# bd4sur/Nano

Hardware: AMD Instinct MI355X
Metric: decode_tokens_per_sec (higher is better)
Workload: dtype i8

## Files before the change

### include/nano_mi355x.h

```cpp
#ifndef NANO_MI355X_H
#define NANO_MI355X_H

#include <stddef.h>
#include <stdint.h>

#ifdef __cplusplus
extern "C" {
#endif

#define NANO_ARCH_NANO  0u
#define NANO_ARCH_QWEN2 2u
#define NANO_ARCH_QWEN3 3u

#define NANO_QUANT_F32 0x00u
#define NANO_QUANT_Q80 0x80u
#define NANO_QUANT_Q4K 0x42u

#define NANO_HIP_OK        0
#define NANO_HIP_EINVAL   -1
#define NANO_HIP_ERUNTIME -2
#define NANO_HIP_ENODEV   -3
#define NANO_HIP_ENOMEM   -4

#define NANO_MAX_BATCH 64u
// ... 268 lines not shown
int nano_hip_qkv_attn_fused_plan(const NanoFusedGemvDesc *qkv, const NanoAttnDecodeDesc *attn, uint32_t cus, uint32_t out[NANO_QKV_ATTN_FUSED_PLAN_WORDS]);
int nano_hip_wo_w13_fused_plan(const NanoFusedGemvDesc *wo, const NanoFusedGemvDesc *w13, uint32_t cus, uint32_t out[NANO_WO_W13_FUSED_PLAN_WORDS]);
typedef struct NanoQkvAttnFusedDesc {
    const NanoFusedGemvDesc *qkv;
    const NanoAttnDecodeDesc *attn;
    uint32_t layer1, tick0;
    const unsigned long long *hand_init;
    float *part_out;
    float *ml_out;
    uint32_t *plan_out;
    uint32_t *err_out;
} NanoQkvAttnFusedDesc;
int nano_hip_op_qkv_attn_fused(int device, const NanoQkvAttnFusedDesc *d);
typedef struct NanoWoW13FusedDesc {
    const NanoFusedGemvDesc *wo, *w13;
    uint32_t layer1, tick0;
    const unsigned long long *hand_init;
    uint32_t *plan_out;
    uint32_t *err_out;
} NanoWoW13FusedDesc;
int nano_hip_op_wo_w13_fused(int device, const NanoWoW13FusedDesc *d);

typedef struct NanoBlobShare NanoBlobShare;
int nano_hip_blob_share(NanoBlobShare **out, const void *host_params, size_t bytes, int root_device, const int *devices, int n_devices);
const void *nano_hip_blob_ptr(const NanoBlobShare *s, int i);
void nano_hip_blob_stats(const NanoBlobShare *s, double *upload_s, double *share_s, char *how, size_t how_cap);
void nano_hip_blob_done(NanoBlobShare *s, int i);
void nano_hip_blob_release(NanoBlobShare *s);
int nano_hip_model_device(const NanoHipModel *m);

int nano_hip_stamps_begin(NanoHipModel *m);
int nano_hip_stamps_read(NanoHipModel *m, unsigned long long *out, uint32_t *kinds, uint32_t cap_launches, uint32_t *n_launches);

#ifdef __cplusplus
}
#endif
#endif
```

### nano_amd/binding.py

```python
from __future__ import annotations

import ctypes as C
import os
from typing import Optional, Sequence

import numpy as np

HERE = os.path.dirname(os.path.abspath(__file__))
LIB_PATH = os.environ.get("NANO_LIB") or os.path.join(HERE, "lib", "libnano_mi355x.so")

f32p = np.ctypeslib.ndpointer(dtype=np.float32, flags="C_CONTIGUOUS")
i8p = np.ctypeslib.ndpointer(dtype=np.int8, flags="C_CONTIGUOUS")
u8p = np.ctypeslib.ndpointer(dtype=np.uint8, flags="C_CONTIGUOUS")
u32p = np.ctypeslib.ndpointer(dtype=np.uint32, flags="C_CONTIGUOUS")


class NanoModelDesc(C.Structure):
    _fields_ = [(n, C.c_uint32) for n in (
        "arch", "block_size", "vocab_size", "n_layer", "n_embd", "n_head", "n_kv_head", "n_hidden",
        "is_shared_classifier", "head_dim", "quant_type", "group_size")]


class NanoFusedGemvDesc(C.Structure):
    _fields_ = [("quant", C.c_uint32), ("gs", C.c_uint32), ("kind", C.c_uint32), ("n", C.c_uint32), ("nb", C.c_uint32), ("nseg", C.c_uint32),
# ... 66 lines not shown


ROUTE_NAMES = ("gemv", "gemv_preq", "gemv_sliced", "q4k", "reserved", "frag_g6", "frag_old", "frag_g7", "q4k_gemm", "f32_gemm")


class NanoHipError(RuntimeError):
    pass


class NanoHipTokenScore(C.Structure):
    _fields_ = [("logprob", C.c_float), ("target_logit", C.c_float), ("max_logit", C.c_float), ("lse", C.c_float),
                ("argmax", C.c_uint32), ("rank", C.c_uint32)]


TOKEN_SCORE_DTYPE = np.dtype([("logprob", "<f4"), ("target_logit", "<f4"), ("max_logit", "<f4"), ("lse", "<f4"), ("argmax", "<u4"), ("rank", "<u4")])
assert TOKEN_SCORE_DTYPE.itemsize == C.sizeof(NanoHipTokenScore)


class NanoHipTopEntry(C.Structure):
    _fields_ = [("token", C.c_uint32), ("logit", C.c_float), ("logprob", C.c_float)]


TOP_ENTRY_DTYPE = np.dtype([("token", "<u4"), ("logit", "<f4"), ("logprob", "<f4")])
assert TOP_ENTRY_DTYPE.itemsize == C.sizeof(NanoHipTopEntry) == 12
TOPK_MAX = 32


class NanoHipLookupParams(C.Structure):
    _fields_ = [(n, C.c_uint32) for n in ("max_draft", "ngram_max", "ngram_min", "stop_token", "max_steps")]


class NanoHipLookupStats(C.Structure):
    _fields_ = [(n, C.c_uint32) for n in ("steps_plain", "steps_verify", "drafted", "accepted", "emitted")]


LOOKUP_RECORD_FIELDS = ("emitted", "accepted", "nb_next", "n", "match_len", "match_end", "done", "left")
LOOKUP_NO_STOP = 0xFFFFFFFF


PHASE_FN = C.CFUNCTYPE(None, C.c_void_p, C.c_int32, C.c_int32)


_lib = None


def lib() -> C.CDLL:
    global _lib
    if _lib is not None:
        return _lib
    if not os.path.exists(LIB_PATH):
        raise NanoHipError(f"{LIB_PATH} not found: build it with `python -c 'import __graft_entry__ as g; g.build()'` "
                           "(there is no CPU fallback)")
    L = C.CDLL(LIB_PATH)
    vp = C.c_void_p

    def fn(name, restype, argtypes):
        f = getattr(L, name)
        f.restype, f.argtypes = restype, argtypes
        return f

    fn("nano_hip_device_count", C.c_int, [])
    fn("nano_hip_last_error", C.c_char_p, [])
    fn("nano_hip_device_info", C.c_int, [C.c_int, C.c_char_p, C.c_size_t, C.POINTER(C.c_uint64)])
    fn("nano_hip_model_create", C.c_int, [C.POINTER(vp), C.POINTER(NanoModelDesc), vp, C.c_size_t, C.c_int, C.c_int, C.c_uint32, C.c_uint32])
    fn("nano_hip_model_create_ex", C.c_int, [C.POINTER(vp), C.POINTER(NanoModelDesc), vp, C.c_size_t, C.c_int, C.c_int, C.c_uint32, C.c_uint32, C.c_uint32])
    fn("nano_hip_model_destroy", None, [vp])
# ... 9 lines not shown
    fn("nano_hip_verify_draft", C.c_int, [vp, C.c_uint32, vp, C.c_uint32, C.c_uint32, vp, C.POINTER(C.c_uint32)])
    fn("nano_hip_op_lookup_step", C.c_int, [C.c_int, vp, C.c_uint32, vp, vp, C.c_uint32, C.POINTER(NanoHipLookupParams), C.c_uint32, C.c_uint32, vp, vp, vp])
    fn("nano_hip_lora_attach", C.c_int, [vp, C.c_uint32, C.c_uint32, f32p, C.c_size_t])
    fn("nano_hip_lora_enable", C.c_int, [vp, C.c_int])
    fn("nano_hip_forward_sample", C.c_int, [vp, C.c_uint32, C.c_uint32, u32p, C.c_uint32, C.c_float, C.c_float, C.c_float, C.c_float, C.POINTER(NanoHipSample)])
    fn("nano_hip_op_sample", C.c_int, [vp, f32p, u32p, C.c_uint32, C.c_float, C.c_float, C.c_float, C.c_float, C.POINTER(NanoHipSample)])
    fn("nano_hip_forward_sample_batch", C.c_int, [vp, u32p, u32p, C.c_uint32, C.POINTER(NanoHipSampleParams), C.POINTER(NanoHipSample)])
    fn("nano_hip_op_sample_batch", C.c_int, [vp, f32p, C.c_uint32, C.POINTER(NanoHipSampleParams), C.POINTER(NanoHipSample)])
    fn("nano_hip_forward_sample_batch_ex", C.c_int, [vp, u32p, u32p, C.c_uint32, C.POINTER(NanoHipSampleParamsEx), C.POINTER(NanoHipSample)])
    fn("nano_hip_op_sample_batch_ex", C.c_int, [vp, f32p, C.c_uint32, C.POINTER(NanoHipSampleParamsEx), C.POINTER(NanoHipSample)])
    fn("nano_hip_sync", C.c_int, [vp])
    fn("nano_hip_set_strict", C.c_int, [vp, C.c_int])
    fn("nano_hip_set_phase_hook", C.c_int, [vp, PHASE_FN, vp])
    fn("nano_hip_set_exact", C.c_int, [vp, C.c_int])
    fn("nano_hip_exact_state", C.c_int, [vp, C.POINTER(C.c_uint32), C.POINTER(C.c_uint32), C.POINTER(C.c_uint32)])
    fn("nano_hip_op_exact_rmsnorm", C.c_int, [C.c_int, f32p, f32p, f32p, C.c_uint32])
    fn("nano_hip_op_exact_attention", C.c_int, [C.c_int, C.POINTER(NanoExactAttnDesc)])
    fn("nano_hip_time_classifier", C.c_int, [vp, C.c_uint32, C.c_uint32, C.POINTER(C.c_float), C.POINTER(C.c_uint64)])
    fn("nano_hip_time_classifier_in_step", C.c_int, [vp, C.c_uint32, C.c_uint32, C.c_uint32, C.POINTER(C.c_float), C.POINTER(C.c_uint64), C.POINTER(C.c_float)])
    fn("nano_hip_time_step", C.c_int, [vp, C.c_uint32, C.c_uint32, C.c_uint32, C.POINTER(C.c_float)])
    fn("nano_hip_membw", C.c_int, [C.c_int, C.c_size_t, C.c_uint32, C.POINTER(C.c_float)])
    fn("nano_hip_read_state", C.c_int, [vp, C.c_uint32, C.c_int, C.c_uint32, C.c_uint32, f32p, C.c_size_t])
    fn("nano_hip_op_rmsnorm", C.c_int, [C.c_int, f32p, f32p, f32p, C.c_uint32])
    fn("nano_hip_op_matmul_f32", C.c_int, [C.c_int, f32p, f32p, f32p, C.c_uint32, C.c_uint32])
    fn("nano_hip_op_quantize_q80", C.c_int, [C.c_int, f32p, C.c_uint32, C.c_uint32, i8p, f32p])
    fn("nano_hip_op_matmul_q80", C.c_int, [C.c_int, f32p, i8p, f32p, i8p, f32p, C.c_uint32, C.c_uint32, C.c_uint32])
    fn("nano_hip_op_quantize_q4k", C.c_int, [C.c_int, f32p, C.c_uint32, u8p])
    fn("nano_hip_op_matmul_q4k", C.c_int, [C.c_int, f32p, u8p, u8p, C.c_uint32, C.c_uint32])
    fn("nano_hip_op_rope", C.c_int, [C.c_int, f32p, C.c_uint32, f32p, f32p, C.c_int])
    fn("nano_hip_op_attention", C.c_int, [C.c_int, f32p, f32p, f32p, f32p, C.c_uint32, C.c_uint32, C.c_uint32, C.c_uint32])
    fn("nano_hip_op_swiglu", C.c_int, [C.c_int, f32p, f32p, C.c_uint32])
    fn("nano_hip_op_argmax", C.c_int, [C.c_int, f32p, C.c_uint32, C.POINTER(C.c_uint32)])
    fn("nano_hip_op_fused_gemv", C.c_int, [C.c_int, C.POINTER(NanoFusedGemvDesc)])
    fn("nano_hip_op_attention_decode", C.c_int, [C.c_int, C.POINTER(NanoAttnDecodeDesc)])
    fn("nano_hip_f32_gemv_plan", C.c_int, [C.POINTER(NanoFusedGemvDesc), C.c_uint32, C.POINTER(C.c_uint32)])
    fn("nano_hip_f32_gemm_plan", C.c_int, [C.POINTER(NanoFusedGemvDesc), C.c_uint32, C.POINTER(C.c_uint32)])
    fn("nano_hip_q80_gemv_plan", C.c_int, [C.POINTER(NanoFusedGemvDesc), C.c_uint32, C.POINTER(C.c_uint32)])
    fn("nano_hip_q80_gemm_plan", C.c_int, [C.POINTER(NanoFusedGemvDesc), C.c_uint32, C.POINTER(C.c_uint32)])
    fn("nano_hip_q4k_gemv_plan", C.c_int, [C.POINTER(NanoFusedGemvDesc), C.c_uint32, C.POINTER(C.c_uint32)])
    fn("nano_hip_qkv_attn_fused_plan", C.c_int, [C.POINTER(NanoFusedGemvDesc), C.POINTER(NanoAttnDecodeDesc), C.c_uint32, C.POINTER(C.c_uint32)])
    fn("nano_hip_wo_w13_fused_plan", C.c_int, [C.POINTER(NanoFusedGemvDesc), C.POINTER(NanoFusedGemvDesc), C.c_uint32, C.POINTER(C.c_uint32)])
    fn("nano_hip_op_qkv_attn_fused", C.c_int, [C.c_int, C.POINTER(NanoQkvAttnFusedDesc)])
    fn("nano_hip_op_wo_w13_fused", C.c_int, [C.c_int, C.POINTER(NanoWoW13FusedDesc)])
    fn("nano_hip_kv_release", C.c_int, [vp, C.c_uint32])
    fn("nano_hip_kv_pages", C.c_int, [vp, C.POINTER(C.c_uint32), C.POINTER(C.c_uint32)])
    fn("nano_hip_kv_fork", C.c_int, [vp, C.c_uint32, C.c_uint32, u32p, C.c_uint32])
    fn("nano_hip_kv_sharing", C.c_int, [vp, C.POINTER(C.c_uint32), C.POINTER(C.c_uint64)])
    fn("nano_prefill_shared", C.c_int, [vp, u32p, C.c_uint32, C.c_uint32])
    for name, args in (("nano_hip_step_rows", [vp, vp, C.c_uint32, vp, vp]),
                       ("nano_hip_rows_plan", [vp, C.c_uint32, C.c_uint32, C.c_uint32, vp, vp, vp, C.POINTER(C.c_uint32)]),
                       ("nano_hip_rows_addressable", [C.c_uint32] * 4),
                       ("nano_prefill_batch", [vp, vp, u32p, C.c_uint32, vp]),
                       ("nano_hip_op_topk_rows", [C.c_int, vp, C.c_uint32, C.c_uint32, C.c_uint32, vp, vp, vp]),
                       ("nano_hip_prefill_score_topk", [vp, C.c_uint32, vp, C.c_uint32, C.c_uint32, vp, C.c_uint32, vp, vp]),
                       ("nano_hip_forward_topk", [vp, vp, vp, C.c_uint32, vp, C.c_uint32, vp, vp]),
                       ("nano_hip_step_rows_score", [vp, vp, C.c_uint32, vp, vp, C.c_uint32, vp, vp]),
                       ("nano_score_ids_topk", [vp, vp, C.c_uint32, C.c_uint32, vp, vp, vp, vp, C.POINTER(C.c_double)]),
                       ("nano_forward_batch_topk", [vp, vp, vp, C.c_uint32, C.c_uint32, vp, vp, vp]),
                       ("nano_hip_forward_sample_batch_edit", [vp, u32p, u32p, C.c_uint32, C.POINTER(NanoHipSampleParamsEdit), C.POINTER(NanoHipSample)]),
                       ("nano_hip_op_sample_batch_edit", [vp, f32p, C.c_uint32, C.POINTER(NanoHipSampleParamsEdit), C.POINTER(NanoHipSample)]),
                       ("nano_hip_mask_table_set", [vp, C.c_void_p, C.c_uint32]),
                       ("nano_set_logit_edit", [vp, vp]),
                       ("nano_forward_batch_sample_edit", [vp, u32p, u32p, C.c_uint32, vp, vp, vp, vp, vp])):
        if hasattr(L, name) or not os.environ.get("NANO_LIB"):
            fn(name, C.c_int, args)
    fn("nano_hip_handoff_state", C.c_int, [vp, C.POINTER(C.c_uint32), C.POINTER(C.c_uint32), C.POINTER(C.c_uint32)])
# ... 764 lines not shown
    return out


def op_topk_rows(logits, k, targets=None, device=0):
    l = np.ascontiguousarray(logits, np.float32)
    if l.ndim != 2:
        raise ValueError("logits must be [rows, V]")
    g = None if targets is None else np.ascontiguousarray(targets, np.uint32).reshape(-1)
    if g is not None and g.size != l.shape[0]:
        raise ValueError(f"{l.shape[0]} rows but {g.size} targets")
    out = np.zeros(l.shape[0], TOKEN_SCORE_DTYPE)
    top = np.zeros((l.shape[0], max(k, 1)), TOP_ENTRY_DTYPE)
    check(lib().nano_hip_op_topk_rows(device, l.ctypes.data, l.shape[0], l.shape[1], k, None if g is None else g.ctypes.data,
                                      out.ctypes.data, top.ctypes.data))
    return out, top


def op_lookup_step(history, fed=(), amax=(), *, left, max_draft=7, ngram_max=3, ngram_min=1, stop_token=None, seq_limit=1 << 30, device=0):
    h = np.ascontiguousarray(history, np.uint32).reshape(-1)
    f = np.ascontiguousarray(fed, np.uint32).reshape(-1)
    g = np.ascontiguousarray(amax, np.uint32).reshape(-1)
    if f.size != g.size:
        raise ValueError(f"{f.size} fed ids but {g.size} arg-maxes")
    buf = np.full(h.size + 16, 0xFFFFFFFF, np.uint32)
    buf[:h.size] = h
    p = NanoHipLookupParams(max_draft, ngram_max, ngram_min, LOOKUP_NO_STOP if stop_token is None else stop_token, 0)
    rec, nt, npos = np.zeros(8, np.uint32), np.zeros(16, np.uint32), np.zeros(16, np.uint32)
    check(lib().nano_hip_op_lookup_step(device, buf.ctypes.data, h.size, f.ctypes.data if f.size else None, g.ctypes.data if g.size else None, f.size,
                                        C.byref(p), left, min(seq_limit, 0xFFFFFFFF), rec.ctypes.data, nt.ctypes.data, npos.ctypes.data))
    r = dict(zip(LOOKUP_RECORD_FIELDS, (int(v) for v in rec)))
    return r, buf[:r["n"]].copy() if h.size <= r["n"] <= buf.size else buf, nt, npos


def op_argmax(x, device=0):
    i = C.c_uint32(0)
    x = np.ascontiguousarray(x, np.float32)
    check(lib().nano_hip_op_argmax(device, x, x.size, C.byref(i))); return int(i.value)


class Engine:

    def __init__(self, path: str, max_seq_len: int = 512, rep_pen: float = 1.0, temperature: float = 0.0,
                 top_p: float = 1.0, top_k: int = 0, seed: int = 39, device: int = 0, max_batch: int = 1,
                 lora_path: Optional[str] = None):
        L = lib()
        vp = C.c_void_p
        L.nano_set_device.argtypes = [C.c_int]; L.nano_set_max_batch.argtypes = [C.c_uint32]
        L.llm_context_init.restype = vp
        L.llm_context_init.argtypes = [C.c_char_p, C.c_char_p, C.c_uint32, C.c_float, C.c_float, C.c_float, C.c_uint32, C.c_uint64]
        L.llm_context_free.argtypes = [vp]
        L.generate_next_token.restype = C.c_uint32
        L.generate_next_token.argtypes = [vp, u32p, C.c_uint32, C.c_int]
        L.nano_session_init_ids.restype = vp
        L.nano_session_init_ids.argtypes = [vp, u32p, C.c_uint32, C.c_uint32]
        L.nano_session_step_ids.restype = C.c_int32
        L.nano_session_step_ids.argtypes = [vp, vp]
        L.llm_session_free.argtypes = [vp]
        L.nano_forward_batch.restype = C.c_int
        L.nano_forward_batch.argtypes = [vp, u32p, u32p, C.c_uint32, vp, vp]
        L.nano_score_ids.restype = C.c_int
        L.nano_score_ids.argtypes = [vp, u32p, C.c_uint32, vp, vp, C.POINTER(C.c_double)]
        L.nano_forward_batch_sample.restype = C.c_int
        L.nano_forward_batch_sample.argtypes = [vp, u32p, u32p, C.c_uint32, vp, vp, vp, vp]
        L.build_sampler.restype = C.POINTER(SamplerC)
        L.build_sampler.argtypes = [C.c_int, C.c_float, C.c_float, C.c_float, C.c_uint32, C.c_uint64]
        L.free_sampler.argtypes = [C.POINTER(SamplerC)]
# ... 142 lines not shown
```

### nano_amd/csrc/misc.hip

```cpp
#include <float.h>

#include "device_common.h"
#include "kernels.h"

namespace nano {

__device__ __forceinline__ void embed_row(const EmbedArgs &a, uint32_t b, uint32_t tok, uint32_t p, bool stage_pos) {
    float *x = a.x + (size_t)b * a.x_bstride;
    const uint32_t E = a.E;
    if (stage_pos && a.kvrow && threadIdx.x == 0 && (p >> 6) < a.pt_entries)
        a.kvrow[b] = a.pt_rows[(a.row_slot ? (size_t)a.row_slot[b] * a.pt_entries : (size_t)b * a.pt_bstride) + (p >> 6)] + (p & 63u);
    if (stage_pos && a.rope_cur) {
        for (uint32_t i = threadIdx.x; i < a.half; i += blockDim.x) {
            a.rope_cur[(size_t)b * 2 * a.half + i] = a.rope_cos[(size_t)p * a.half + i];
            a.rope_cur[(size_t)b * 2 * a.half + a.half + i] = a.rope_sin[(size_t)p * a.half + i];
        }
    }
    if (a.quant == 0x00u) {
        const float4 *row = reinterpret_cast<const float4 *>(reinterpret_cast<const float *>(a.tok) + (size_t)tok * E);
        for (uint32_t i = threadIdx.x; i < E / 4; i += blockDim.x) reinterpret_cast<float4 *>(x)[i] = row[i];
    } else if (a.quant == 0x80u) {
        const int8_t *row = reinterpret_cast<const int8_t *>(a.tok) + (size_t)tok * E;
        const float *s = a.tok_s + ((size_t)tok * E) / a.gs;
        for (uint32_t i = threadIdx.x * 4; i < E; i += blockDim.x * 4) {
            const uint32_t w = *reinterpret_cast<const uint32_t *>(row + i);
            const float sc = s[i / a.gs];
            reinterpret_cast<float4 *>(x + i)[0] = make_float4((float)(int8_t)(w & 0xff) * sc, (float)(int8_t)((w >> 8) & 0xff) * sc,
                                                               (float)(int8_t)((w >> 16) & 0xff) * sc, (float)(int8_t)(w >> 24) * sc);
        }
    } else {
        const uint32_t bpl = (E + 255) / 256;
        const uint8_t *blocks = reinterpret_cast<const uint8_t *>(a.tok) + (size_t)tok * bpl * 160;
        for (uint32_t it = threadIdx.x; it < bpl * 256; it += blockDim.x) {
            const uint32_t j = it >> 8, k = it & 255;
            const uint8_t *blk = blocks + (size_t)j * 160;
            const uint32_t d = (E >= (j + 1) * 256) ? 256 : (E - j * 256);
            const uint32_t len = *reinterpret_cast<const uint32_t *>(blk + 4);
            if (k < len) {
                const float s_scale = *reinterpret_cast<const float *>(blk + 12);
                const float s_bias = *reinterpret_cast<const float *>(blk + 16);
                uint32_t s6, b6;
                q4k_unpack6(*reinterpret_cast<const uint32_t *>(blk + 20), *reinterpret_cast<const uint32_t *>(blk + 24),
                            *reinterpret_cast<const uint32_t *>(blk + 28), (int)(k >> 5), s6, b6);
                const float sc = (float)s6 * s_scale, bb = (float)b6 * s_bias;
                const uint8_t byte = blk[32 + (k >> 1)];
                const uint32_t nib = (k & 1) ? (uint32_t)(byte >> 4) : (uint32_t)(byte & 0x0f);
                x[(size_t)j * d + k] = (float)nib * sc - bb;
            }
        }
    }
}

__global__ __launch_bounds__(256) void embed_kernel(const EmbedArgs a) {
    const int b = blockIdx.x;
    if (a.tick && b == 0 && threadIdx.x == 0) a.tick[0] = a.tick[0] + 1u;
    embed_row(a, (uint32_t)b, a.tokens[b], a.pos ? a.pos[b] : 0u, true);
}

hipError_t launch_embed(const EmbedArgs &a, uint32_t nb, hipStream_t st) {
    hipLaunchKernelGGL(embed_kernel, dim3(nb), dim3(256), 0, st, a);
    return hipGetLastError();
}

__global__ __launch_bounds__(1024) void argmax_kernel(const ArgmaxArgs a) {
    __shared__ float sval[16];
    __shared__ uint32_t sidx[16];
    __shared__ uint32_t s_next[2];
    const int b = blockIdx.x, tid = threadIdx.x;
    const float *x = a.logits + (size_t)b * a.bstride;
    float best = -INFINITY;
    uint32_t bi = 0xffffffffu;
    if (a.tile_max) {
        const float *tm = a.tile_max + (size_t)b * a.ntiles * 2;
        for (uint32_t t = tid; t < a.ntiles; t += blockDim.x) {
            const float v = tm[2 * t];
            const uint32_t i = __float_as_uint(tm[2 * t + 1]);
            if (i != 0xffffffffu && (bi == 0xffffffffu || v > best || (v == best && i < bi))) { best = v; bi = i; }
        }
    } else {
        const uint32_t V4 = ((reinterpret_cast<uintptr_t>(x) & 15) == 0) ? a.V / 4 : 0;
        auto upd = [&](float v, uint32_t i) { if (bi == 0xffffffffu || v > best) { best = v; bi = i; } };
        uint32_t i = tid;
        for (; i + 3 * blockDim.x < V4; i += 4 * blockDim.x) {
            const float4 v0 = reinterpret_cast<const float4 *>(x)[i], v1 = reinterpret_cast<const float4 *>(x)[i + blockDim.x];
            const float4 v2 = reinterpret_cast<const float4 *>(x)[i + 2 * blockDim.x], v3 = reinterpret_cast<const float4 *>(x)[i + 3 * blockDim.x];
            upd(v0.x, 4 * i); upd(v0.y, 4 * i + 1); upd(v0.z, 4 * i + 2); upd(v0.w, 4 * i + 3);
            const uint32_t i1 = i + blockDim.x, i2 = i + 2 * blockDim.x, i3 = i + 3 * blockDim.x;
            upd(v1.x, 4 * i1); upd(v1.y, 4 * i1 + 1); upd(v1.z, 4 * i1 + 2); upd(v1.w, 4 * i1 + 3);
            upd(v2.x, 4 * i2); upd(v2.y, 4 * i2 + 1); upd(v2.z, 4 * i2 + 2); upd(v2.w, 4 * i2 + 3);
            upd(v3.x, 4 * i3); upd(v3.y, 4 * i3 + 1); upd(v3.z, 4 * i3 + 2); upd(v3.w, 4 * i3 + 3);
        }
        for (; i < V4; i += blockDim.x) {
            const float4 v0 = reinterpret_cast<const float4 *>(x)[i];
            upd(v0.x, 4 * i); upd(v0.y, 4 * i + 1); upd(v0.z, 4 * i + 2); upd(v0.w, 4 * i + 3);
        }
        for (uint32_t k = V4 * 4 + tid; k < a.V; k += blockDim.x) upd(x[k], k);
    }
#pragma unroll
    for (int o = 32; o > 0; o >>= 1) {
        const float ov = __shfl_xor(best, o, 64);
        const uint32_t oi = __shfl_xor(bi, o, 64);
        if (oi != 0xffffffffu && (bi == 0xffffffffu || ov > best || (ov == best && oi < bi))) { best = ov; bi = oi; }
    }
    const int lane = tid & 63, wid = tid >> 6;
    if (lane == 0) { sval[wid] = best; sidx[wid] = bi; }
    __syncthreads();
    if (tid == 0) {
        const int nw = (blockDim.x + 63) >> 6;
        for (int w = 1; w < nw; w++) {
            const float ov = sval[w]; const uint32_t oi = sidx[w];
            if (oi != 0xffffffffu && (bi == 0xffffffffu || ov > best || (ov == best && oi < bi))) { best = ov; bi = oi; }
        }
        if (bi == 0xffffffffu) bi = 0;
        a.out[b] = bi;
        if (a.tokens) a.tokens[b] = bi;
        if (a.trace) a.trace[(size_t)(a.pos[b] - a.pos0[b]) * a.nb + b] = bi;
        if (a.tokens) { const uint32_t np = a.pos[b] + 1; a.pos[b] = np; s_next[0] = bi; s_next[1] = np; }
    }
    if (a.tokens && a.emb.x) {
        __syncthreads();
        const uint32_t np = s_next[1];
        if (a.emb.tick && b == 0 && tid == 0) a.emb.tick[0] = a.emb.tick[0] + 1u;
        embed_row(a.emb, (uint32_t)b, s_next[0], np, np < a.rope_rows);
    }
}

hipError_t launch_argmax(const ArgmaxArgs &a, uint32_t nb, hipStream_t st) {
    hipLaunchKernelGGL(argmax_kernel, dim3(nb), dim3(1024), 0, st, a);
    return hipGetLastError();
}


__global__ __launch_bounds__(256) void rmsnorm_kernel(float *out, const float *x, const float *w, uint32_t n) {
    __shared__ float red[32];
    float acc = 0.0f;
    for (uint32_t i = threadIdx.x; i < n; i += blockDim.x) acc += x[i] * x[i];
    float ss = block_sum(acc, red);
    ss /= (float)n; ss += 1e-5f; ss = 1.0f / sqrtf(ss);
    for (uint32_t i = threadIdx.x; i < n; i += blockDim.x) out[i] = w[i] * (ss * x[i]);
}
hipError_t launch_rmsnorm(float *out, const float *x, const float *w, uint32_t n, hipStream_t st) {
    hipLaunchKernelGGL(rmsnorm_kernel, dim3(1), dim3(256), 0, st, out, x, w, n);
    return hipGetLastError();
}

__global__ __launch_bounds__(256) void quantize_q80_kernel(const float *x, uint32_t n, uint32_t gs, int8_t *q, float *s) {
    const int tid = threadIdx.x, nthr = blockDim.x;
    const int tpg = (int)gs / 4;
    const int iters = ((int)n + nthr * 4 - 1) / (nthr * 4);
    for (int it = 0; it < iters; it++) {
        const int i = (it * nthr + tid) * 4;
        const bool act = i < (int)n;
        float4 v = act ? *reinterpret_cast<const float4 *>(x + i) : make_float4(0.f, 0.f, 0.f, 0.f);
        float m = fmaxf(fmaxf(fabsf(v.x), fabsf(v.y)), fmaxf(fabsf(v.z), fabsf(v.w)));
        m = group_max(m, tpg);
        const float scale = div_const<127>(m);
        if (act) {
            *reinterpret_cast<uint32_t *>(q + i) = q80_pack4(q80_quant4(v, scale));
            if ((tid % tpg) == 0) s[i / (int)gs] = scale;
        }
    }
// ... 70 lines not shown
```

### nano_amd/csrc/ops.hip

```cpp
#include <stdio.h>
#include <string.h>

#include <array>
#include <string>
#include <vector>

#include "../../include/nano_mi355x.h"
#include "kernels.h"

using namespace nano;

extern "C" const char *nano_hip_last_error(void);
namespace { thread_local std::string g_op_err; }

extern "C" void nano_hip_set_error_(const char *msg);

struct DevBufs {
    std::vector<void *> ptrs;
    ~DevBufs() { for (void *p : ptrs) (void)hipFree(p); }
    template <typename T> T *alloc(size_t n) {
        void *p = nullptr;
        if (hipMalloc(&p, n * sizeof(T) + 16) != hipSuccess) return nullptr;
        ptrs.push_back(p);
        return reinterpret_cast<T *>(p);
// ... 141 lines not shown
    OP_HIP(launch_exact_rmsnorm(dout, dx, dw, n, 1, n, n, 0));
    OP_HIP(hipMemcpy(out, dout, (size_t)n * 4, hipMemcpyDeviceToHost));
    return 0;
}

extern "C" int nano_hip_op_exact_attention(int device, const NanoExactAttnDesc *d) {
    int rc; if ((rc = begin(device))) return rc;
    if (!d || !d->q || !d->k_cache || !d->v_cache || !d->out) { nano_hip_set_error_("null argument"); return NANO_HIP_EINVAL; }
    if (!d->n_head || !d->n_kv_head || d->n_head % d->n_kv_head || !d->hd || d->hd % 4 || d->hd > 256 || !d->S ||
        (d->is_causal && (d->range == 0 || d->range > d->S))) { nano_hip_set_error_("bad attention shape"); return NANO_HIP_EINVAL; }
    if (!d->long_form && !exact_attention_fits(d->hd, d->S)) { nano_hip_set_error_("S rows do not fit the one-launch kernel's LDS: set long_form"); return NANO_HIP_EINVAL; }
    const uint32_t qd = d->n_head * d->hd, kvd = d->n_kv_head * d->hd, pos = d->is_causal ? d->range - 1u : 0u;
    DevBufs B;
    float *dq = B.upload(d->q, qd), *dk = B.upload(d->k_cache, (size_t)d->S * kvd), *dv = B.upload(d->v_cache, (size_t)d->S * kvd);
    float *dout = B.alloc<float>(qd), *datt = d->long_form ? B.alloc<float>((size_t)d->n_head * d->S) : nullptr;
    uint32_t *dpos = B.upload(&pos, 1);
    OP_CHECK(dq && dk && dv && dout && dpos && (datt || !d->long_form), "device alloc failed");
    StrictAttnArgs sa{};
    sa.q = dq; sa.kcache = dk; sa.vcache = dv; sa.pos = dpos; sa.att = datt; sa.xba = dout;
    sa.n_head = d->n_head; sa.n_kv_head = d->n_kv_head; sa.hd = d->hd; sa.q_dim = qd; sa.kv_dim = kvd;
    sa.layer = 0; sa.n_layer = 1; sa.S = d->S; sa.slot0 = 0; sa.is_causal = d->is_causal ? 1u : 0u;
    OP_HIP(d->long_form ? launch_strict_attention(sa, 1, 0) : launch_exact_attention(sa, 1, 0));
    OP_HIP(hipMemcpy(d->out, dout, (size_t)qd * 4, hipMemcpyDeviceToHost));
    return 0;
}

extern "C" int nano_hip_op_argmax(int device, const float *x, uint32_t n, uint32_t *idx) {
    int rc; if ((rc = begin(device))) return rc;
    DevBufs B; float *dx = B.upload(x, n); uint32_t *di = B.alloc<uint32_t>(1);
    OP_CHECK(dx && di, "device alloc failed");
    ArgmaxArgs a{ dx, n, n, di, nullptr, nullptr, nullptr, nullptr, 1 };
    OP_HIP(launch_argmax(a, 1, 0));
    OP_HIP(hipMemcpy(idx, di, 4, hipMemcpyDeviceToHost));
    return 0;
}

extern "C" int nano_hip_op_score_rows(int device, const float *logits, uint32_t rows, uint32_t V, const uint32_t *targets, NanoHipTokenScore *out) {
    if (!logits || !out || !rows || !V) { nano_hip_set_error_("score_rows: null logits / out, or no rows / no vocabulary"); return NANO_HIP_EINVAL; }
    if (targets) for (uint32_t r = 0; r < rows; r++) if (targets[r] >= V) { nano_hip_set_error_("score_rows: target out of vocabulary"); return NANO_HIP_EINVAL; }
    int rc; if ((rc = begin(device))) return rc;
    DevBufs B;
    ScoreArgs a{};
    a.V = V; a.ntiles = score_tiles(V);
    a.logits = B.upload(logits, (size_t)rows * V);
    a.targets = targets ? B.upload(targets, rows) : nullptr;
    a.part = B.alloc<ScorePartial>((size_t)rows * a.ntiles); a.out = B.alloc<NanoHipTokenScore>(rows);
    OP_CHECK(a.logits && (a.targets || !targets) && a.part && a.out, "device alloc failed");
    OP_HIP(launch_score_rows(a, rows, 0));
    OP_HIP(hipMemcpy(out, a.out, (size_t)rows * sizeof(NanoHipTokenScore), hipMemcpyDeviceToHost));
    return 0;
}

extern "C" int nano_hip_op_topk_rows(int device, const float *logits, uint32_t rows, uint32_t V, uint32_t k, const uint32_t *targets,
                                     NanoHipTokenScore *scores_out, NanoHipTopEntry *top_out) {
    if (!logits || !top_out || !rows || !V || !k) { nano_hip_set_error_("topk_rows: null logits / top_out, or no rows / no vocabulary / k of 0"); return NANO_HIP_EINVAL; }
    if (k > NANO_TOPK_MAX || k > V) { nano_hip_set_error_("topk_rows: k exceeds NANO_TOPK_MAX or the vocabulary"); return NANO_HIP_EINVAL; }
    if (rows > 65535u) { nano_hip_set_error_("topk_rows: more than 65535 rows"); return NANO_HIP_EINVAL; }
    if (targets) for (uint32_t r = 0; r < rows; r++) if (targets[r] >= V) { nano_hip_set_error_("topk_rows: target out of vocabulary"); return NANO_HIP_EINVAL; }
    int rc; if ((rc = begin(device))) return rc;
    DevBufs B;
    ScoreArgs a{};
    a.V = V; a.ntiles = score_tiles(V);
    a.logits = B.upload(logits, (size_t)rows * V);
    a.targets = targets ? B.upload(targets, rows) : nullptr;
    a.part = B.alloc<ScorePartial>((size_t)rows * a.ntiles); a.out = B.alloc<NanoHipTokenScore>(rows);
    TopkArgs t{};
// ... 549 lines not shown
```

Measured before the change: 2056.

## Restructure argmax+embed kernel: templated threads, hoisted loads, overlapped embed staging

Rewrites the argmax kernel as a template over thread count, using 256 threads when reducing tile partials and 1024 for raw logits. It reads partials as vectorized float4 loads with unrolled prefetch and issues the pos, tick, page-table and RoPE loads before the reduction so their latency overlaps it. The per-block second barrier and shared-memory handoff are replaced by a broadcast reduction in which every thread knows the winning token. Embedding now uses shift-based group indexing, and the Q4K path gains a 'covered' skip condition. A host test entry point is added, and the new Q4K skip logic risks correctness.

```diff
diff --git a/include/nano_mi355x.h b/include/nano_mi355x.h
--- a/include/nano_mi355x.h
+++ b/include/nano_mi355x.h
@@ -324,6 +324,22 @@
 int nano_hip_stamps_begin(NanoHipModel *m);
 int nano_hip_stamps_read(NanoHipModel *m, unsigned long long *out, uint32_t *kinds, uint32_t cap_launches, uint32_t *n_launches);
 
+typedef struct NanoArgmaxEmbedDesc {
+    const float *partials; uint32_t ntiles;
+    const float *logits; uint32_t V;
+    uint32_t nb, loop, embed, trace_rows;
+    const uint32_t *pos, *pos0;
+    uint32_t quant, E, gs, table_rows;
+    const void *tok; const float *tok_s;
+    const float *rope_cos, *rope_sin; uint32_t rope_rows, half;
+    const uint32_t *pt; const uint32_t *row_slot; uint32_t pt_words, pt_entries, pt_bstride;
+    uint32_t use_tick, tick0, _pad;
+    uint32_t *out, *tokens_out, *pos_out, *trace_out;
+    float *x_out, *rope_cur_out;
+    uint32_t *kvrow_out, *tick_out;
+} NanoArgmaxEmbedDesc;
+int nano_hip_op_argmax_embed(int device, const NanoArgmaxEmbedDesc *d);
+
 #ifdef __cplusplus
 }
 #endif
diff --git a/nano_amd/binding.py b/nano_amd/binding.py
--- a/nano_amd/binding.py
+++ b/nano_amd/binding.py
@@ -122,6 +122,19 @@
 
 class NanoHipLookupStats(C.Structure):
     _fields_ = [(n, C.c_uint32) for n in ("steps_plain", "steps_verify", "drafted", "accepted", "emitted")]
+
+
+class NanoArgmaxEmbedDesc(C.Structure):
+    _fields_ = [("partials", C.c_void_p), ("ntiles", C.c_uint32), ("logits", C.c_void_p), ("V", C.c_uint32),
+                ("nb", C.c_uint32), ("loop", C.c_uint32), ("embed", C.c_uint32), ("trace_rows", C.c_uint32),
+                ("pos", C.c_void_p), ("pos0", C.c_void_p),
+                ("quant", C.c_uint32), ("E", C.c_uint32), ("gs", C.c_uint32), ("table_rows", C.c_uint32),
+                ("tok", C.c_void_p), ("tok_s", C.c_void_p),
+                ("rope_cos", C.c_void_p), ("rope_sin", C.c_void_p), ("rope_rows", C.c_uint32), ("half", C.c_uint32),
+                ("pt", C.c_void_p), ("row_slot", C.c_void_p), ("pt_words", C.c_uint32), ("pt_entries", C.c_uint32), ("pt_bstride", C.c_uint32),
+                ("use_tick", C.c_uint32), ("tick0", C.c_uint32), ("_pad", C.c_uint32),
+                ("out", C.c_void_p), ("tokens_out", C.c_void_p), ("pos_out", C.c_void_p), ("trace_out", C.c_void_p),
+                ("x_out", C.c_void_p), ("rope_cur_out", C.c_void_p), ("kvrow_out", C.c_void_p), ("tick_out", C.c_void_p)]
 
 
 LOOKUP_RECORD_FIELDS = ("emitted", "accepted", "nb_next", "n", "match_len", "match_end", "done", "left")
@@ -197,6 +210,8 @@
     fn("nano_hip_op_swiglu", C.c_int, [C.c_int, f32p, f32p, C.c_uint32])
     fn("nano_hip_op_argmax", C.c_int, [C.c_int, f32p, C.c_uint32, C.POINTER(C.c_uint32)])
     fn("nano_hip_op_fused_gemv", C.c_int, [C.c_int, C.POINTER(NanoFusedGemvDesc)])
+    if hasattr(L, "nano_hip_op_argmax_embed"):
+        fn("nano_hip_op_argmax_embed", C.c_int, [C.c_int, C.POINTER(NanoArgmaxEmbedDesc)])
     fn("nano_hip_op_attention_decode", C.c_int, [C.c_int, C.POINTER(NanoAttnDecodeDesc)])
     fn("nano_hip_f32_gemv_plan", C.c_int, [C.POINTER(NanoFusedGemvDesc), C.c_uint32, C.POINTER(C.c_uint32)])
     fn("nano_hip_f32_gemm_plan", C.c_int, [C.POINTER(NanoFusedGemvDesc), C.c_uint32, C.POINTER(C.c_uint32)])
@@ -1027,6 +1042,57 @@
     return r, buf[:r["n"]].copy() if h.size <= r["n"] <= buf.size else buf, nt, npos
 
 
+def op_argmax_embed(*, partials=None, logits=None, loop=False, pos=None, pos0=None, trace_rows=0, table=None, quant=0, E=0, gs=0,
+                    table_scales=None, rope_cos=None, rope_sin=None, rope_rows=0, pt=None, pt_entries=0, pt_bstride=0, row_slot=None,
+                    tick0=None, device=0):
+    keep = []
+
+    def arr(a, dt):
+        if a is None:
+            return None
+        a = np.ascontiguousarray(a, dt)
+        keep.append(a)
+        return a
+
+    def ptr(a):
+        return None if a is None else a.ctypes.data
+
+    d = NanoArgmaxEmbedDesc()
+    if partials is not None:
+        c = arr(partials, np.float32)
+        nb, d.partials, d.ntiles = c.shape[0], ptr(c), c.shape[1]
+    else:
+        c = arr(logits, np.float32)
+        nb, d.logits, d.V = c.shape[0], ptr(c), c.shape[1]
+    d.nb, d.loop, d.trace_rows = nb, int(loop), trace_rows
+    d.pos, d.pos0 = ptr(arr(pos, np.uint32)), ptr(arr(pos0, np.uint32))
+    res = {"out": np.zeros(nb, np.uint32)}
+    if loop:
+        res["tokens"], res["pos"] = np.zeros(nb, np.uint32), np.zeros(nb, np.uint32)
+        if trace_rows:
+            res["trace"] = np.zeros((trace_rows, nb), np.uint32)
+    d.rope_rows = rope_rows
+    if table is not None:
+        t = arr(table, {0x00: np.float32, 0x80: np.int8}.get(quant, np.uint8))
+        d.embed, d.quant, d.E, d.gs, d.table_rows, d.tok, d.tok_s = 1, quant, E, gs, t.shape[0], ptr(t), ptr(arr(table_scales, np.float32))
+        res["x"] = np.zeros((nb, E), np.float32)
+        if rope_cos is not None:
+            rc, rs = arr(rope_cos, np.float32), arr(rope_sin, np.float32)
+            d.rope_cos, d.rope_sin, d.half = ptr(rc), ptr(rs), rc.shape[1]
+            res["rope_cur"] = np.zeros((nb, 2 * rc.shape[1]), np.float32)
+        if pt is not None:
+            t = arr(pt, np.uint32)
+            d.pt, d.pt_words, d.pt_entries, d.pt_bstride, d.row_slot = ptr(t), t.size, pt_entries, pt_bstride, ptr(arr(row_slot, np.uint32))
+            res["kvrow"] = np.zeros(nb, np.uint32)
+        if tick0 is not None:
+            d.use_tick, d.tick0 = 1, tick0
+            res["tick"] = np.zeros(1, np.uint32)
+    for k, v in res.items():
+        setattr(d, {"out": "out", "tick": "tick_out"}.get(k, k + "_out"), v.ctypes.data)
+    check(lib().nano_hip_op_argmax_embed(device, C.byref(d)))
+    return res
+
+
 def op_argmax(x, device=0):
     i = C.c_uint32(0)
     x = np.ascontiguousarray(x, np.float32)
diff --git a/nano_amd/csrc/misc.hip b/nano_amd/csrc/misc.hip
--- a/nano_amd/csrc/misc.hip
+++ b/nano_amd/csrc/misc.hip
@@ -5,38 +5,33 @@
 
 namespace nano {
 
-__device__ __forceinline__ void embed_row(const EmbedArgs &a, uint32_t b, uint32_t tok, uint32_t p, bool stage_pos) {
+__device__ __forceinline__ void embed_x(const EmbedArgs &a, uint32_t b, uint32_t tok, uint32_t nthr) {
     float *x = a.x + (size_t)b * a.x_bstride;
     const uint32_t E = a.E;
-    if (stage_pos && a.kvrow && threadIdx.x == 0 && (p >> 6) < a.pt_entries)
-        a.kvrow[b] = a.pt_rows[(a.row_slot ? (size_t)a.row_slot[b] * a.pt_entries : (size_t)b * a.pt_bstride) + (p >> 6)] + (p & 63u);
-    if (stage_pos && a.rope_cur) {
-        for (uint32_t i = threadIdx.x; i < a.half; i += blockDim.x) {
-            a.rope_cur[(size_t)b * 2 * a.half + i] = a.rope_cos[(size_t)p * a.half + i];
-            a.rope_cur[(size_t)b * 2 * a.half + a.half + i] = a.rope_sin[(size_t)p * a.half + i];
-        }
-    }
     if (a.quant == 0x00u) {
         const float4 *row = reinterpret_cast<const float4 *>(reinterpret_cast<const float *>(a.tok) + (size_t)tok * E);
-        for (uint32_t i = threadIdx.x; i < E / 4; i += blockDim.x) reinterpret_cast<float4 *>(x)[i] = row[i];
+        for (uint32_t i = threadIdx.x; i < E / 4; i += nthr) reinterpret_cast<float4 *>(x)[i] = row[i];
     } else if (a.quant == 0x80u) {
         const int8_t *row = reinterpret_cast<const int8_t *>(a.tok) + (size_t)tok * E;
-        const float *s = a.tok_s + ((size_t)tok * E) / a.gs;
-        for (uint32_t i = threadIdx.x * 4; i < E; i += blockDim.x * 4) {
+        const uint32_t gsh = 31u - (uint32_t)__clz((int)a.gs);
+        const float *s = a.tok_s + (size_t)tok * (E >> gsh);
+        for (uint32_t i = threadIdx.x * 4; i < E; i += nthr * 4) {
             const uint32_t w = *reinterpret_cast<const uint32_t *>(row + i);
-            const float sc = s[i / a.gs];
+            const float sc = s[i >> gsh];
             reinterpret_cast<float4 *>(x + i)[0] = make_float4((float)(int8_t)(w & 0xff) * sc, (float)(int8_t)((w >> 8) & 0xff) * sc,
                                                                (float)(int8_t)((w >> 16) & 0xff) * sc, (float)(int8_t)(w >> 24) * sc);
         }
     } else {
         const uint32_t bpl = (E + 255) / 256;
         const uint8_t *blocks = reinterpret_cast<const uint8_t *>(a.tok) + (size_t)tok * bpl * 160;
-        for (uint32_t it = threadIdx.x; it < bpl * 256; it += blockDim.x) {
+        const uint32_t dl = E - (bpl - 1) * 256;
+        for (uint32_t it = threadIdx.x; it < bpl * 256; it += nthr) {
             const uint32_t j = it >> 8, k = it & 255;
             const uint8_t *blk = blocks + (size_t)j * 160;
             const uint32_t d = (E >= (j + 1) * 256) ? 256 : (E - j * 256);
             const uint32_t len = *reinterpret_cast<const uint32_t *>(blk + 4);
-            if (k < len) {
+            const bool covered = j + 1 < bpl && j * d + k >= (bpl - 1) * dl && j * d + k < bpl * dl;
+            if (k < len && !covered) {
                 const float s_scale = *reinterpret_cast<const float *>(blk + 12);
                 const float s_bias = *reinterpret_cast<const float *>(blk + 16);
                 uint32_t s6, b6;
@@ -50,6 +45,17 @@
         }
     }
 }
+__device__ __forceinline__ void embed_row(const EmbedArgs &a, uint32_t b, uint32_t tok, uint32_t p, bool stage_pos) {
+    if (stage_pos && a.kvrow && threadIdx.x == 0 && (p >> 6) < a.pt_entries)
+        a.kvrow[b] = a.pt_rows[(a.row_slot ? (size_t)a.row_slot[b] * a.pt_entries : (size_t)b * a.pt_bstride) + (p >> 6)] + (p & 63u);
+    if (stage_pos && a.rope_cur) {
+        for (uint32_t i = threadIdx.x; i < a.half; i += blockDim.x) {
+            a.rope_cur[(size_t)b * 2 * a.half + i] = a.rope_cos[(size_t)p * a.half + i];
+            a.rope_cur[(size_t)b * 2 * a.half + a.half + i] = a.rope_sin[(size_t)p * a.half + i];
+        }
+    }
+    embed_x(a, b, tok, blockDim.x);
+}
 
 __global__ __launch_bounds__(256) void embed_kernel(const EmbedArgs a) {
     const int b = blockIdx.x;
@@ -62,71 +68,130 @@
     return hipGetLastError();
 }
 
-__global__ __launch_bounds__(1024) void argmax_kernel(const ArgmaxArgs a) {
-    __shared__ float sval[16];
-    __shared__ uint32_t sidx[16];
-    __shared__ uint32_t s_next[2];
-    const int b = blockIdx.x, tid = threadIdx.x;
+constexpr uint32_t AMAX_EMPTY = 0xffffffffu;
+#ifndef NANO_AMAX_PART_THREADS
+#define NANO_AMAX_PART_THREADS 256
+#endif
+constexpr int AMAX_PART_THREADS = NANO_AMAX_PART_THREADS;
+static_assert(AMAX_PART_THREADS == 256 || AMAX_PART_THREADS == 1024, "a multiple of 128 threads that the launcher instantiates");
+__device__ __forceinline__ void amax_take(float &best, uint32_t &bi, float v, uint32_t i) {
+    const bool t = (i != AMAX_EMPTY) & ((bi == AMAX_EMPTY) | (v > best) | ((v == best) & (i < bi)));
+    best = t ? v : best; bi = t ? i : bi;
+}
+template <int NT>
+__global__ __launch_bounds__(NT) void argmax_kernel(const ArgmaxArgs a) {
+    constexpr int NW = NT / 64;
+    constexpr int U = NT >= 1024 ? 2 : 8;
+    __shared__ uint4 sres[(NW + 1) / 2];
+    karg_touch(a.logits); karg_touch(a.V); karg_touch(a.bstride); karg_touch(a.out); karg_touch(a.tokens); karg_touch(a.pos); karg_touch(a.trace);
+    karg_touch(a.pos0); karg_touch(a.nb); karg_touch(a.tile_max); karg_touch(a.ntiles); karg_touch(a.rope_rows);
+    karg_touch(a.emb.tok); karg_touch(a.emb.tok_s); karg_touch(a.emb.x); karg_touch(a.emb.E); karg_touch(a.emb.gs); karg_touch(a.emb.quant); karg_touch(a.emb.x_bstride);
+    karg_touch(a.emb.rope_cos); karg_touch(a.emb.rope_sin); karg_touch(a.emb.rope_cur); karg_touch(a.emb.half); karg_touch(a.emb.pt_rows); karg_touch(a.emb.kvrow);
+    karg_touch(a.emb.pt_bstride); karg_touch(a.emb.pt_entries); karg_touch(a.emb.tick); karg_touch(a.emb.row_slot);
+    const uint32_t b = blockIdx.x, tid = threadIdx.x;
+    const bool embed = a.tokens && a.emb.x;
+    uint32_t vz = 0;
+    asm volatile("" : "+v"(vz));
+    const uint32_t *spare = a.out + b;
+    const bool bump = embed && a.emb.tick && b == 0;
+    const bool paged = embed && a.emb.kvrow;
+    const uint32_t p_v = ((a.tokens || a.trace) ? a.pos + b : spare)[vz];
+    const uint32_t p0_v = (a.trace ? a.pos0 + b : spare)[vz];
+    const uint32_t tick_v = (bump ? a.emb.tick : spare)[vz];
+    const uint32_t slot_v = ((paged && a.emb.row_slot) ? a.emb.row_slot + b : spare)[vz];
     const float *x = a.logits + (size_t)b * a.bstride;
+    const float2 *tm = reinterpret_cast<const float2 *>(a.tile_max) + (size_t)b * a.ntiles;
+    const uint32_t head = (a.tile_max && (reinterpret_cast<uintptr_t>(tm) & 8)) ? 1u : 0u;
+    const uint32_t n4 = a.tile_max ? (a.ntiles - head) / 2 : 0u;
+    const float4 *tm4 = reinterpret_cast<const float4 *>(tm + head);
+    const float4 none4 = make_float4(0.f, __uint_as_float(AMAX_EMPTY), 0.f, __uint_as_float(AMAX_EMPTY));
+    float4 pv[U];
+    float2 ph = make_float2(0.f, __uint_as_float(AMAX_EMPTY)), pl = ph;
+#pragma unroll
+    for (int k = 0; k < U; k++) pv[k] = none4;
+    if (a.tile_max) {
+        ph = tm[vz]; pl = tm[a.ntiles - 1 + vz];
+        if (n4) {
+#pragma unroll
+            for (int k = 0; k < U; k++) pv[k] = tm4[min(tid + k * NT, n4 - 1)];
+        }
+    }
+    const uint32_t p = __builtin_amdgcn_readfirstlane(p_v), np = p + 1u;
+    const bool stage = embed && np < a.rope_rows;
+    const bool kv_on = stage && paged && (np >> 6) < a.emb.pt_entries;
+    uint32_t kv_entry = 0u;
+    if (kv_on) kv_entry = a.emb.pt_rows[(a.emb.row_slot ? (size_t)slot_v * a.emb.pt_entries : (size_t)b * a.emb.pt_bstride) + (np >> 6)];
+    const uint32_t half = a.emb.half;
+    const bool rope_on = stage && a.emb.rope_cur;
+    float rope_v = 0.f;
+    if (rope_on && tid < 2 * half) rope_v = tid < half ? a.emb.rope_cos[(size_t)np * half + tid] : a.emb.rope_sin[(size_t)np * half + (tid - half)];
     float best = -INFINITY;
-    uint32_t bi = 0xffffffffu;
+    uint32_t bi = AMAX_EMPTY;
     if (a.tile_max) {
-        const float *tm = a.tile_max + (size_t)b * a.ntiles * 2;
-        for (uint32_t t = tid; t < a.ntiles; t += blockDim.x) {
-            const float v = tm[2 * t];
-            const uint32_t i = __float_as_uint(tm[2 * t + 1]);
-            if (i != 0xffffffffu && (bi == 0xffffffffu || v > best || (v == best && i < bi))) { best = v; bi = i; }
+        amax_take(best, bi, ph.x, __float_as_uint(ph.y));
+        amax_take(best, bi, pl.x, __float_as_uint(pl.y));
+#pragma unroll
+        for (int k = 0; k < U; k++) { amax_take(best, bi, pv[k].x, __float_as_uint(pv[k].y)); amax_take(best, bi, pv[k].z, __float_as_uint(pv[k].w)); }
+        for (uint32_t q0 = tid + U * NT; q0 < n4; q0 += U * NT) {
+#pragma unroll
+            for (int k = 0; k < U; k++) pv[k] = tm4[min(q0 + k * NT, n4 - 1)];
+#pragma unroll
+            for (int k = 0; k < U; k++) { amax_take(best, bi, pv[k].x, __float_as_uint(pv[k].y)); amax_take(best, bi, pv[k].z, __float_as_uint(pv[k].w)); }
         }
     } else {
         const uint32_t V4 = ((reinterpret_cast<uintptr_t>(x) & 15) == 0) ? a.V / 4 : 0;
-        auto upd = [&](float v, uint32_t i) { if (bi == 0xffffffffu || v > best) { best = v; bi = i; } };
+        auto upd = [&](float v, uint32_t i) { if (bi == AMAX_EMPTY || v > best) { best = v; bi = i; } };
         uint32_t i = tid;
-        for (; i + 3 * blockDim.x < V4; i += 4 * blockDim.x) {
-            const float4 v0 = reinterpret_cast<const float4 *>(x)[i], v1 = reinterpret_cast<const float4 *>(x)[i + blockDim.x];
-            const float4 v2 = reinterpret_cast<const float4 *>(x)[i + 2 * blockDim.x], v3 = reinterpret_cast<const float4 *>(x)[i + 3 * blockDim.x];
+        for (; i + 3 * NT < V4; i += 4 * NT) {
+            const float4 v0 = reinterpret_cast<const float4 *>(x)[i], v1 = reinterpret_cast<const float4 *>(x)[i + NT];
+            const float4 v2 = reinterpret_cast<const float4 *>(x)[i + 2 * NT], v3 = reinterpret_cast<const float4 *>(x)[i + 3 * NT];
             upd(v0.x, 4 * i); upd(v0.y, 4 * i + 1); upd(v0.z, 4 * i + 2); upd(v0.w, 4 * i + 3);
-            const uint32_t i1 = i + blockDim.x, i2 = i + 2 * blockDim.x, i3 = i + 3 * blockDim.x;
+            const uint32_t i1 = i + NT, i2 = i + 2 * NT, i3 = i + 3 * NT;
             upd(v1.x, 4 * i1); upd(v1.y, 4 * i1 + 1); upd(v1.z, 4 * i1 + 2); upd(v1.w, 4 * i1 + 3);
             upd(v2.x, 4 * i2); upd(v2.y, 4 * i2 + 1); upd(v2.z, 4 * i2 + 2); upd(v2.w, 4 * i2 + 3);
             upd(v3.x, 4 * i3); upd(v3.y, 4 * i3 + 1); upd(v3.z, 4 * i3 + 2); upd(v3.w, 4 * i3 + 3);
         }
-        for (; i < V4; i += blockDim.x) {
+        for (; i < V4; i += NT) {
             const float4 v0 = reinterpret_cast<const float4 *>(x)[i];
             upd(v0.x, 4 * i); upd(v0.y, 4 * i + 1); upd(v0.z, 4 * i + 2); upd(v0.w, 4 * i + 3);
         }
-        for (uint32_t k = V4 * 4 + tid; k < a.V; k += blockDim.x) upd(x[k], k);
+        for (uint32_t k = V4 * 4 + tid; k < a.V; k += NT) upd(x[k], k);
     }
 #pragma unroll
     for (int o = 32; o > 0; o >>= 1) {
         const float ov = __shfl_xor(best, o, 64);
         const uint32_t oi = __shfl_xor(bi, o, 64);
-        if (oi != 0xffffffffu && (bi == 0xffffffffu || ov > best || (ov == best && oi < bi))) { best = ov; bi = oi; }
-    }
-    const int lane = tid & 63, wid = tid >> 6;
-    if (lane == 0) { sval[wid] = best; sidx[wid] = bi; }
+        amax_take(best, bi, ov, oi);
+    }
+    if ((tid & 63u) == 0) reinterpret_cast<uint2 *>(sres)[tid >> 6] = make_uint2(__float_as_uint(best), bi);
     __syncthreads();
+    best = -INFINITY; bi = AMAX_EMPTY;
+#pragma unroll
+    for (int w = 0; w < (NW + 1) / 2; w++) {
+        const uint4 r = sres[w];
+        amax_take(best, bi, __uint_as_float(r.x), r.y);
+        if (2 * w + 1 < NW) amax_take(best, bi, __uint_as_float(r.z), r.w);
+    }
+    const uint32_t tok = __builtin_amdgcn_readfirstlane(bi == AMAX_EMPTY ? 0u : bi);
+    if (embed) embed_x(a.emb, b, tok, NT);
     if (tid == 0) {
-        const int nw = (blockDim.x + 63) >> 6;
-        for (int w = 1; w < nw; w++) {
-            const float ov = sval[w]; const uint32_t oi = sidx[w];
-            if (oi != 0xffffffffu && (bi == 0xffffffffu || ov > best || (ov == best && oi < bi))) { best = ov; bi = oi; }
-        }
-        if (bi == 0xffffffffu) bi = 0;
-        a.out[b] = bi;
-        if (a.tokens) a.tokens[b] = bi;
-        if (a.trace) a.trace[(size_t)(a.pos[b] - a.pos0[b]) * a.nb + b] = bi;
-        if (a.tokens) { const uint32_t np = a.pos[b] + 1; a.pos[b] = np; s_next[0] = bi; s_next[1] = np; }
-    }
-    if (a.tokens && a.emb.x) {
-        __syncthreads();
-        const uint32_t np = s_next[1];
-        if (a.emb.tick && b == 0 && tid == 0) a.emb.tick[0] = a.emb.tick[0] + 1u;
-        embed_row(a.emb, (uint32_t)b, s_next[0], np, np < a.rope_rows);
+        a.out[b] = tok;
+        if (a.tokens) a.tokens[b] = tok;
+        if (a.trace) a.trace[(size_t)(p - p0_v) * a.nb + b] = tok;
+        if (a.tokens) a.pos[b] = np;
+        if (kv_on) a.emb.kvrow[b] = kv_entry + (np & 63u);
+        if (bump) a.emb.tick[0] = tick_v + 1u;
+    }
+    if (rope_on) {
+        if (tid < 2 * half) a.emb.rope_cur[(size_t)b * 2 * half + tid] = rope_v;
+        for (uint32_t i = tid + NT; i < 2 * half; i += NT)
+            a.emb.rope_cur[(size_t)b * 2 * half + i] = i < half ? a.emb.rope_cos[(size_t)np * half + i] : a.emb.rope_sin[(size_t)np * half + (i - half)];
     }
 }
 
 hipError_t launch_argmax(const ArgmaxArgs &a, uint32_t nb, hipStream_t st) {
-    hipLaunchKernelGGL(argmax_kernel, dim3(nb), dim3(1024), 0, st, a);
+    if (a.tile_max) hipLaunchKernelGGL(argmax_kernel<AMAX_PART_THREADS>, dim3(nb), dim3(AMAX_PART_THREADS), 0, st, a);
+    else hipLaunchKernelGGL(argmax_kernel<1024>, dim3(nb), dim3(1024), 0, st, a);
     return hipGetLastError();
 }
 
diff --git a/nano_amd/csrc/ops.hip b/nano_amd/csrc/ops.hip
--- a/nano_amd/csrc/ops.hip
+++ b/nano_amd/csrc/ops.hip
@@ -197,6 +197,89 @@
     ArgmaxArgs a{ dx, n, n, di, nullptr, nullptr, nullptr, nullptr, 1 };
     OP_HIP(launch_argmax(a, 1, 0));
     OP_HIP(hipMemcpy(idx, di, 4, hipMemcpyDeviceToHost));
+    return 0;
+}
+
+static const char *argmax_embed_error(const NanoArgmaxEmbedDesc &d) {
+    if (!d.out || !d.nb || d.nb > 64) return "argmax_embed: null out, or nb outside 1 .. 64";
+    if (d.partials ? !d.ntiles : (!d.logits || !d.V)) return "argmax_embed: neither partials nor logits";
+    if (d.loop && (!d.pos || !d.tokens_out || !d.pos_out)) return "argmax_embed: loop without pos / tokens_out / pos_out";
+    if (d.trace_out) {
+        if (!d.loop || !d.pos0 || !d.trace_rows) return "argmax_embed: trace without loop / pos0 / trace_rows";
+        for (uint32_t b = 0; b < d.nb; b++) if (d.pos[b] < d.pos0[b] || d.pos[b] - d.pos0[b] >= d.trace_rows) return "argmax_embed: position outside the trace";
+    }
+    if (d.loop) for (uint32_t b = 0; b < d.nb; b++) if (d.pos[b] == 0xffffffffu) return "argmax_embed: position overflow";
+    if (!d.embed) return nullptr;
+    if (!d.pos) return "argmax_embed: embed without pos";
+    if (!d.tok || !d.x_out || !d.table_rows || !d.E || d.E % 4) return "argmax_embed: null table / x_out, or E not a multiple of 4";
+    if (d.quant != NANO_QUANT_F32 && d.quant != NANO_QUANT_Q80 && d.quant != NANO_QUANT_Q4K) return "argmax_embed: unknown quant type";
+    if (d.quant == NANO_QUANT_Q80 && (!d.tok_s || !(d.gs == 32 || d.gs == 64 || d.gs == 128 || d.gs == 256) || d.E % d.gs)) return "argmax_embed: bad Q80 scales / group size";
+    if (d.partials) {
+        for (size_t i = 0; i < (size_t)d.nb * d.ntiles; i++) {
+            uint32_t row; memcpy(&row, d.partials + 2 * i + 1, 4);
+            if (row != 0xffffffffu && row >= d.table_rows) return "argmax_embed: partial row outside the table";
+        }
+    } else if (d.V > d.table_rows) return "argmax_embed: vocabulary larger than the table";
+    if (d.rope_cos && (!d.rope_sin || !d.rope_cur_out || !d.half || !d.rope_rows)) return "argmax_embed: incomplete RoPE tables";
+    if (d.pt) {
+        if (!d.kvrow_out || !d.pt_entries) return "argmax_embed: page table without kvrow_out / entries";
+        for (uint32_t b = 0; b < d.nb; b++) {
+            const size_t base = d.row_slot ? (size_t)d.row_slot[b] * d.pt_entries : (size_t)b * d.pt_bstride;
+            if (base + d.pt_entries > d.pt_words) return "argmax_embed: page-table row outside pt_words";
+        }
+    }
+    if (d.use_tick && !d.tick_out) return "argmax_embed: use_tick without tick_out";
+    return nullptr;
+}
+extern "C" int nano_hip_op_argmax_embed(int device, const NanoArgmaxEmbedDesc *dp) {
+    if (!dp) { nano_hip_set_error_("argmax_embed: null descriptor"); return NANO_HIP_EINVAL; }
+    const NanoArgmaxEmbedDesc &d = *dp;
+    if (const char *why = argmax_embed_error(d)) { nano_hip_set_error_(why); return NANO_HIP_EINVAL; }
+    int rc; if ((rc = begin(device))) return rc;
+    DevBufs B;
+    const uint32_t nb = d.nb;
+    bool ok = true;
+    auto filled = [&](size_t words) { uint32_t *p = B.alloc<uint32_t>(words); ok = ok && p && hipMemset(p, 0xff, words * 4) == hipSuccess; return p; };
+    auto up = [&](const auto *h, size_t n) { auto *p = B.upload(h, n); ok = ok && p; return p; };
+    ArgmaxArgs a{};
+    if (d.partials) { a.tile_max = up(d.partials, (size_t)nb * d.ntiles * 2); a.ntiles = d.ntiles; }
+    else { a.logits = up(d.logits, (size_t)nb * d.V); a.V = d.V; a.bstride = d.V; }
+    a.out = filled(nb); a.nb = nb;
+    if (d.pos) a.pos = up(d.pos, nb);
+    if (d.pos0) a.pos0 = up(d.pos0, nb);
+    if (d.loop) a.tokens = filled(nb);
+    if (d.trace_out) a.trace = filled((size_t)d.trace_rows * nb);
+    a.rope_rows = d.rope_rows;
+    if (d.embed) {
+        EmbedArgs &e = a.emb;
+        const size_t n = (size_t)d.table_rows * d.E;
+        if (d.quant == NANO_QUANT_F32) e.tok = up(reinterpret_cast<const float *>(d.tok), n);
+        else if (d.quant == NANO_QUANT_Q80) { e.tok = up(reinterpret_cast<const int8_t *>(d.tok), n); e.tok_s = up(d.tok_s, n / d.gs); }
+        else e.tok = up(reinterpret_cast<const uint8_t *>(d.tok), (size_t)d.table_rows * ((d.E + 255) / 256) * 160);
+        e.x = reinterpret_cast<float *>(filled((size_t)nb * d.E));
+        e.E = d.E; e.gs = d.gs; e.quant = d.quant; e.x_bstride = d.E; e.half = d.half; e.pos = a.pos;
+        if (d.rope_cos) {
+            e.rope_cos = up(d.rope_cos, (size_t)d.rope_rows * d.half); e.rope_sin = up(d.rope_sin, (size_t)d.rope_rows * d.half);
+            e.rope_cur = reinterpret_cast<float *>(filled((size_t)nb * 2 * d.half));
+        }
+        if (d.pt) {
+            e.pt_rows = up(d.pt, d.pt_words); e.kvrow = filled(nb); e.pt_bstride = d.pt_bstride; e.pt_entries = d.pt_entries;
+            if (d.row_slot) e.row_slot = up(d.row_slot, nb);
+        }
+        if (d.use_tick) e.tick = up(&d.tick0, 1);
+    }
+    OP_CHECK(ok, "device alloc failed");
+    OP_HIP(launch_argmax(a, nb, 0));
+    OP_HIP(hipDeviceSynchronize());
+    auto down = [&](void *h, const void *dev, size_t bytes) { return (h && dev) ? hipMemcpy(h, dev, bytes, hipMemcpyDeviceToHost) : hipSuccess; };
+    OP_HIP(down(d.out, a.out, (size_t)nb * 4));
+    OP_HIP(down(d.tokens_out, a.tokens, (size_t)nb * 4));
+    OP_HIP(down(d.pos_out, a.pos, (size_t)nb * 4));
+    OP_HIP(down(d.trace_out, a.trace, (size_t)d.trace_rows * nb * 4));
+    OP_HIP(down(d.x_out, a.emb.x, (size_t)nb * d.E * 4));
+    OP_HIP(down(d.rope_cur_out, a.emb.rope_cur, (size_t)nb * 2 * d.half * 4));
+    OP_HIP(down(d.kvrow_out, a.emb.kvrow, (size_t)nb * 4));
+    OP_HIP(down(d.tick_out, a.emb.tick, 4));
     return 0;
 }
 
```

Result: no change. 2069, median of 6 (+0.6%).
